# churchill-lab/gbrs

Measured on AMD Instinct MI355X. Metric: EM iterations/s (EMASE Model 4, 40M reads x 8 haplotypes x 120k isoforms per GPU), higher is better.
Workload: dtype f64

## Files before the change

### gbrs_amd/_lib.py

```python
from __future__ import annotations

import ctypes as C
import os

_HERE = os.path.dirname(os.path.abspath(__file__))
LIB_PATH = os.environ.get("GBRS_TUNING_LIB") or os.path.join(_HERE, "libgbrs_hip.so")

EXPORTS = [
    "gbrs_last_error", "gbrs_abi_version", "gbrs_device_count", "gbrs_warm_up",
    "gbrs_em_create", "gbrs_em_create_device", "gbrs_em_create_masked", "gbrs_em_create_masked_device", "gbrs_em_set_initial_values", "gbrs_em_prepare", "gbrs_em_step", "gbrs_em_run",
    "gbrs_em_set_groups", "gbrs_em_step_model", "gbrs_em_posterior",
    "gbrs_em_resample", "gbrs_em_weights", "gbrs_em_resample_info",
    "gbrs_em_bootstrap_begin", "gbrs_em_bootstrap_add", "gbrs_em_bootstrap_get",
    "gbrs_em_get", "gbrs_em_set_theta", "gbrs_em_group_sums", "gbrs_em_estep_partial",
    "gbrs_em_finish_step", "gbrs_em_prepare_partial", "gbrs_em_finish_prepare", "gbrs_em_stream",
    "gbrs_em_set_stream",
    "gbrs_em_sync", "gbrs_em_pair_begin", "gbrs_em_pair_check", "gbrs_em_pair_status", "gbrs_em_info", "gbrs_em_fold_counts", "gbrs_em_tile_cut", "gbrs_em_gather_mstep", "gbrs_em_tile_shapes",
    "gbrs_alignment_counts",
    "gbrs_counts_create", "gbrs_counts_get", "gbrs_counts_destroy", "gbrs_em_destroy",
    "gbrs_shard_plan", "gbrs_shard_index", "gbrs_shard_gather",
    "gbrs_hmm_create", "gbrs_hmm_set_expression", "gbrs_hmm_set_eprob", "gbrs_hmm_run",
    "gbrs_hmm_get", "gbrs_hmm_info", "gbrs_hmm_destroy",
    "gbrs_grid_knots", "gbrs_hmm_set_grid", "gbrs_hmm_grid", "gbrs_hmm_grid_info", "gbrs_hmm_sample_paths", "gbrs_hmm_sample_info",
    "gbrs_hmm_diagnostics", "gbrs_hmm_pair_posterior", "gbrs_hmm_diagnostics_info",
    "gbrs_hmm_set_panel", "gbrs_hmm_match", "gbrs_hmm_match_info",
    "gbrs_hmm_set_snps", "gbrs_hmm_impute", "gbrs_hmm_impute_info", "gbrs_hmm_impute_times",
    "gbrs_hmm_loglik", "gbrs_hmm_loglik_tables", "gbrs_hmm_loglik_info", "gbrs_interpolate", "gbrs_genoprob_dosage",
    "gbrs_ri_transition_tables", "gbrs_alignment_spec",
    "gbrs_scan_create", "gbrs_scan_destroy", "gbrs_scan_append", "gbrs_scan_append_hmm", "gbrs_scan_prepare", "gbrs_scan_run",
    "gbrs_scan_info", "gbrs_scan_permute", "gbrs_scan_perm_info",
    "gbrs_scan_set_snps", "gbrs_scan_snp_dosage", "gbrs_scan_snps", "gbrs_scan_snp_info",
    "gbrs_scan_mediate", "gbrs_scan_mediate_info",
    "gbrs_scan_effects", "gbrs_scan_effects_info", "gbrs_scan_run_support",
    "gbrs_compress_create", "gbrs_compress_get", "gbrs_compress_destroy",
    "gbrs_bam_open", "gbrs_bam_references", "gbrs_bam_set_reference_map", "gbrs_bam_convert", "gbrs_bam_get",
    "gbrs_bam_scan_records", "gbrs_bam_destroy",
    "gbrs_ecset_create", "gbrs_ecset_add_bam", "gbrs_ecset_add_bam_pair", "gbrs_ecset_sizes", "gbrs_ecset_get", "gbrs_ecset_destroy",
    "gbrs_matops_create", "gbrs_matops_intersect", "gbrs_matops_append_rows", "gbrs_matops_keep_unique_rows",
    "gbrs_matops_mask_columns", "gbrs_matops_sizes", "gbrs_matops_get", "gbrs_matops_destroy",
    "gbrs_matops_shared_counts", "gbrs_matops_shared_counts_get", "gbrs_matops_shared_counts_info",
# ... 134 lines not shown
        "gbrs_em_resample": [vp, u64, u32],
        "gbrs_em_weights": [vp, vp],
        "gbrs_em_resample_info": [vp, C.POINTER(u64), C.POINTER(u64), C.POINTER(u32)],
        "gbrs_em_bootstrap_begin": [vp, i64, vp, vp],
        "gbrs_em_bootstrap_add": [vp, vp, vp, vp, vp],
        "gbrs_em_bootstrap_get": [vp, i32, C.POINTER(u32), vp, vp, vp, vp, vp, vp, vp, vp],
        "gbrs_em_get": [vp, vp, vp],
        "gbrs_em_set_theta": [vp, vp],
        "gbrs_em_group_sums": [vp, i64, vp, vp, i32, vp],
        "gbrs_em_estep_partial": [vp, pp, C.POINTER(u64)],
        "gbrs_em_finish_step": [vp, C.POINTER(dbl)],
        "gbrs_em_prepare_partial": [vp, pp, C.POINTER(u64)],
        "gbrs_em_finish_prepare": [vp, dbl],
        "gbrs_em_sync": [vp],
        "gbrs_em_pair_begin": [vp, vp, i32],
        "gbrs_em_pair_check": [vp, vp, dbl],
        "gbrs_em_pair_status": [vp, vp, C.POINTER(i32), C.POINTER(i32), vp, i32],
        "gbrs_em_set_stream": [vp, vp],
        "gbrs_em_info": [vp, C.POINTER(EmInfo)],
        "gbrs_em_fold_counts": [vp, C.POINTER(u64), C.POINTER(u64)],
        "gbrs_em_tile_cut": [vp, C.POINTER(u32), C.POINTER(u32)],
        "gbrs_em_gather_mstep": [vp, C.POINTER(u32)],
        "gbrs_em_tile_shapes": [vp, vp, vp, u64],
        "gbrs_alignment_counts": [u64, u32, u32, pp, pp, vp, vp, u32, i32, vp, vp, vp],
        "gbrs_counts_create": [u64, u32, u32, pp, pp, vp, i32, pp],
        "gbrs_counts_get": [vp, vp, u32, vp, vp, vp],
        "gbrs_counts_destroy": [vp],
        "gbrs_em_destroy": [vp],
        "gbrs_shard_plan": [u64, u32, u32, pp, pp, i32, i32, vp],
        "gbrs_shard_index": [u64, u32, u32, pp, pp, u64, u64, i32, pp, vp],
        "gbrs_shard_gather": [u64, u32, u32, pp, pp, u64, u64, u32, pp, i32, vp, pp, pp, C.POINTER(u64)],
        "gbrs_hmm_create": [i32, i32, vp, vp, pp, i32, pp],
        "gbrs_hmm_set_expression": [vp, i32, pp, pp, pp, dbl, dbl],
        "gbrs_hmm_set_eprob": [vp, i32, pp],
        "gbrs_hmm_run": [vp],
        "gbrs_hmm_get": [vp, i32, i32, vp, vp, vp, vp, vp, vp, vp, vp],
        "gbrs_hmm_info": [vp, C.POINTER(HmmInfo)],
        "gbrs_hmm_destroy": [vp],
        "gbrs_grid_knots": [i32, vp, i32, vp, vp, vp],
        "gbrs_hmm_set_grid": [vp, vp, pp, vp, pp],
        "gbrs_hmm_grid": [vp, i32, vp, vp],
        "gbrs_hmm_grid_info": [vp, C.POINTER(i64), C.POINTER(dbl)],
        "gbrs_hmm_set_panel": [vp, i32, pp],
        "gbrs_hmm_match": [vp, i32, vp, vp],
        "gbrs_hmm_match_info": [vp, C.POINTER(i32), vp, C.POINTER(dbl), C.POINTER(u64)],
        "gbrs_hmm_set_snps": [vp, vp, pp, vp, pp, pp],
# ... 49 lines not shown
        "gbrs_matops_sizes": [vp, C.POINTER(u64), vp, C.POINTER(u32)],
        "gbrs_matops_get": [vp, pp, pp],
        "gbrs_matops_destroy": [vp],
        "gbrs_matops_shared_counts": [vp, vp, u32, C.POINTER(u64)],
        "gbrs_matops_shared_counts_get": [vp, vp, vp, vp],
        "gbrs_matops_shared_counts_info": [vp, C.POINTER(u64), C.POINTER(u64), C.POINTER(u64), C.POINTER(u32),
                                           C.POINTER(u64), C.POINTER(u64), C.POINTER(dbl)],
        "gbrs_tensor_create": [u64, u32, u32, pp, pp, pp, vp, i32, pp],
        "gbrs_tensor_set_groups": [vp, i64, vp, vp],
        "gbrs_tensor_reset": [vp],
        "gbrs_tensor_multiply": [vp, i32, vp, u64],
        "gbrs_tensor_multiply_tensor": [vp, vp],
        "gbrs_tensor_normalize": [vp, i32],
        "gbrs_tensor_sum_reads": [vp, vp],
        "gbrs_tensor_sum_loci": [vp, vp],
        "gbrs_tensor_copy": [vp, pp],
        "gbrs_tensor_values": [vp, u32, vp, vp, u64],
        "gbrs_tensor_set_values": [vp, u32, vp, u64],
        "gbrs_tensor_nnz": [vp, vp],
        "gbrs_tensor_destroy": [vp],
    }
    sigs.update(_host_signatures())
    for name, args in sigs.items():
        if name in ("gbrs_em_fold_counts", "gbrs_em_tile_cut", "gbrs_em_gather_mstep", "gbrs_em_tile_shapes") and os.environ.get("GBRS_TUNING_LIB") and not hasattr(lib, name):
            continue
        fn = getattr(lib, name)
        fn.restype = i32
        fn.argtypes = args
    lib.gbrs_em_stream.restype = vp
    lib.gbrs_em_stream.argtypes = [vp]
    if lib.gbrs_abi_version() != 5:
        raise ImportError("libgbrs_hip.so ABI version mismatch")
    _lib = lib
    return lib


def _host_signatures():
    vp, i32, u32, u64, i64, dbl = C.c_void_p, C.c_int, C.c_uint32, C.c_uint64, C.c_int64, C.c_double
    return {
        "gbrs_format_double": [dbl, C.c_char_p],
        "gbrs_decode_chunks": [C.c_char_p, i64, vp, vp, vp, vp, u64, u32, u64, i32, i32, vp, i32],
        "gbrs_inflate_backend": [],
        "gbrs_zip_directory": [vp, u64, u64, vp, vp, vp, vp, vp, vp, u64, C.POINTER(u64), C.POINTER(u64)],
        "gbrs_npz_stack": [vp, u64, i64, vp, vp, vp, vp, vp, vp, u64, u64, vp, vp, i32],
        "gbrs_zip_read_members": [vp, u64, i64, vp, vp, vp, vp, vp, vp, i32],
        "gbrs_parse_number_table": [C.c_char_p, i64, i64, i32, vp],
        "gbrs_parse_length_table": [C.c_char_p, i64, C.c_char_p, vp, i64, C.c_char_p, vp, i32, dbl, vp],
# ... 52 lines not shown
```

### gbrs_amd/csrc/em.hip

```cpp
#include "common.h"
#include "em_layout.h"
#include "em_step.h"

#include <algorithm>
#include <chrono>
#include <cmath>
#include <cstdlib>

namespace gbrs {


struct EmScalars {
    double s_prev, s_new;
    double err_sum;
    double pc_before, pc_after;
    int stop;
    int iters_done;
    int float_error;
    int ticket;
};

constexpr int RED_BLOCKS = 256;
constexpr int RED_THREADS = 256;

// ... 1915 lines not shown
    *tile_words = em->layout == 1 ? em->tl.cut_tile_words : 0;
    return GBRS_OK;
}

int gbrs_em_gather_mstep(gbrs_em_t *em, uint32_t *taken) {
    if (!em || !taken) return fail(GBRS_ERR_INVALID, "NULL argument");
    *taken = em_gather_route(em) ? 1u : 0u;
    return GBRS_OK;
}

int gbrs_em_tile_shapes(gbrs_em_t *em, uint32_t *n_batches, uint32_t *dict_entries, uint64_t n) {
    if (!em || !n_batches || !dict_entries) return fail(GBRS_ERR_INVALID, "NULL argument");
    if (em->layout != 1 || n != em->tl.n_tiles) return fail(GBRS_ERR_INVALID, "n is not the handle's number of tiles");
    (void)hipSetDevice(em->device);
    std::vector<TileHdr> hdr(n);
    if (n) GBRS_HIP_CHECK(hipMemcpy(hdr.data(), em->tl.tiles.p, n * sizeof(TileHdr), hipMemcpyDeviceToHost));
    for (uint64_t t = 0; t < n; ++t) {
        n_batches[t] = hdr[t].n_batches;
        dict_entries[t] = hdr[t].dict_count();
    }
    return GBRS_OK;
}

int gbrs_counts_create(uint64_t R, uint32_t L, uint32_t H, const uint32_t *const *indptr,
                       const uint32_t *const *indices, const double *count, int device, gbrs_counts_t **out) {
    if (!out) return fail(GBRS_ERR_INVALID, "out is NULL");
    *out = nullptr;
    if (H < 1 || H > 32 || L < 1 || R < 1 || R > 0xFFFFFFFFull || !indptr || !indices)
        return fail(GBRS_ERR_INVALID, "The shape must be a tuple of three positive integers (H <= 32, R < 2^32).");
    GBRS_TRY(select_device(device));
    gbrs_counts *c = new gbrs_counts();
    struct Guard { gbrs_counts *p; ~Guard() { if (p) gbrs_counts_destroy(p); } } guard{c};
    c->device = device;
    c->R = R; c->L = L; c->H = H;
    GBRS_HIP_CHECK(hipStreamCreateWithFlags(&c->s, hipStreamDefault));
    GBRS_TRY(upload_csc(R, L, H, indptr, indices, false, c->ent_row, c->col_ptr, c->n));
    if (count) {
        GBRS_TRY(c->d_count.alloc(R));
        GBRS_HIP_CHECK(hipMemcpy(c->d_count.p, count, R * sizeof(double), hipMemcpyHostToDevice));
    }
    GBRS_HIP_CHECK(hipDeviceSynchronize());
    GBRS_TRY(check_row_ids(c->n, c->ent_row.p, R, c->s));
    c->work = counts_work_new();
    guard.p = nullptr;
    *out = c;
    return GBRS_OK;
// ... 226 lines not shown
```

### gbrs_amd/csrc/em_layout.h

```cpp
#pragma once
#include "common.h"
#include "em_plan.h"

#include <vector>

namespace gbrs {

#ifndef GBRS_TILE_THREADS
#define GBRS_TILE_THREADS 512
#endif
constexpr int TILE_THREADS = GBRS_TILE_THREADS;
constexpr int TILE_WAVES = TILE_THREADS / 64;
#ifndef GBRS_TILE_CAP
#define GBRS_TILE_CAP 32768
#endif
#ifndef GBRS_TILE_WORDS
#define GBRS_TILE_WORDS 2048
#endif
constexpr int TILE_WORDS = GBRS_TILE_WORDS, TILE_WORDS_MAX = GBRS_TILE_CAP - 64, TILE_ROUNDS_MIN = 1;
static_assert(TILE_WORDS <= TILE_WORDS_MAX, "a tile's padded words must fit the dictionary sort");
__host__ __device__ constexpr int pos_bits(int H) { return H <= 8 ? 5 : 3; }
__host__ __device__ constexpr int max_row_words(int H) { return 1 << pos_bits(H); }
#ifndef GBRS_LDS_DOUBLES
#define GBRS_LDS_DOUBLES 3072
// ... 45 lines not shown
    double *theta_new;
    double *tot_prev, *tot_new;
    double *msums;
    uint32_t cap;
    double *acc_cur, *acc_next;
    const uint32_t *gdest, *gdest_b, *gdest_list;
    uint32_t pending;
};

struct TileLayout {
    uint64_t n_pairs = 0;
    uint64_t n_rows_in = 0;
    uint64_t n_rows = 0;
    uint64_t n_folded = 0;
    uint64_t n_folded_two = 0;
    uint64_t n_long = 0;
    uint64_t n_tiles = 0, n_batches = 0, n_slots = 0, n_heavy = 0, n_light = 0;
    uint32_t d_max = 0;
    uint32_t cut_passes = 0;
    uint32_t cut_tile_words = 0;
    bool weighted = false;
    bool deterministic = false;
    bool all_one_word = false;

    DevBuf<uint32_t> words;
    DevBuf<TileHdr> tiles;
    DevBuf<uint32_t> dict;
    DevBuf<double> word_weight;
    DevBuf<double> row_weight;
    DevBuf<uint32_t> slot_ptr;
    DevBuf<uint32_t> slot_list;
    DevBuf<uint32_t> heavy_loci;
    DevBuf<uint32_t> light_loci;
    DevBuf<uint32_t> heavy_range, light_range;
    DevBuf<uint32_t> slot_dest;
    DevBuf<uint8_t> locus_class;
    DevBuf<double> partials;
    DevBuf<uint64_t> long_ptr;
    DevBuf<uint32_t> long_loc, long_mask;
    DevBuf<double> long_weight;
    DevBuf<double> acc_extra;
    bool keep_row_ids = false;
    DevBuf<uint32_t> word_row;
    DevBuf<uint32_t> long_row;
    uint32_t n_sets = 0;
    uint64_t n_dest_rows = 0;
// ... 87 lines not shown
```

### gbrs_amd/csrc/em_layout.hip

```cpp
#include "em_layout.h"
#include "prim.h"

#include <algorithm>

namespace gbrs {
namespace {



struct BuildFlags {
    unsigned int duplicate;
    unsigned int dict_overflow;
    unsigned int bad_row;
    unsigned int n_long;
    unsigned int long_pairs;
};

constexpr int KEY_ITERS = 32, KEY_SPAN = 64 * KEY_ITERS;
__global__ void __launch_bounds__(256)
make_keys_kernel(uint64_t n, uint32_t ncols, uint32_t L, uint64_t R, unsigned row_shift,
                 const uint64_t *__restrict__ col_ptr, const uint32_t *__restrict__ ent_row,
                 uint64_t *__restrict__ keys, BuildFlags *flags, uint32_t view_h = 0) {
    const int lane = threadIdx.x & 63;
    const uint64_t base = ((uint64_t)blockIdx.x * 4 + (threadIdx.x >> 6)) * KEY_SPAN;
// ... 513 lines not shown

__global__ void permute_rows_kernel(uint64_t m_rows, const uint32_t *__restrict__ perm, const uint32_t *__restrict__ hrow,
                                    const uint32_t *__restrict__ npm, const double *__restrict__ weight,
                                    const uint32_t *__restrict__ repeat, uint32_t *__restrict__ hrow2,
                                    uint32_t *__restrict__ npm2, double *__restrict__ weight2,
                                    uint32_t *__restrict__ repeat2) {
    const uint64_t i = (uint64_t)blockIdx.x * blockDim.x + threadIdx.x;
    if (i >= m_rows) return;
    const uint32_t m = perm[i];
    hrow2[i] = hrow[m];
    npm2[i] = npm[m];
    if (weight) weight2[i] = weight[m];
    if (repeat) repeat2[i] = repeat[m];
}

__global__ void tile_start_kernel(uint64_t m_rows, uint64_t n_tiles, const uint32_t *__restrict__ tflag,
                                  const uint32_t *__restrict__ tincl, uint32_t *__restrict__ tile_row) {
    const uint64_t m = (uint64_t)blockIdx.x * blockDim.x + threadIdx.x;
    if (m == 0) tile_row[n_tiles] = (uint32_t)m_rows;
    if (m >= m_rows || !tflag[m]) return;
    tile_row[tincl[m] - 1] = (uint32_t)m;
}

__global__ void tile_pad_kernel(uint64_t n_tiles, int streams, const uint32_t *__restrict__ tile_row,
                                const uint32_t *__restrict__ npm, uint32_t *__restrict__ rowpad,
                                uint32_t *__restrict__ nbatch, uint32_t *__restrict__ n_one, uint32_t *__restrict__ n_two) {
    const uint64_t t = (uint64_t)blockIdx.x * blockDim.x + threadIdx.x;
    if (t >= n_tiles) return;
    uint32_t off = 0, one = 0, two = 0;
    const uint32_t end = tile_row[t + 1];
    uint32_t m = tile_row[t];
    while (m < end) {
        const uint32_t cnt = npm[m];
        if (streams && cnt <= 32u && (64u % cnt) == 0u) {
            uint32_t e = m + 1;
            while (e < end && npm[e] == cnt) ++e;
            const uint32_t n = e - m, G = 64u / cnt, B = (n + G - 1) / G;
            off = (off + 63u) & ~63u;
            if (cnt == 1u && off == 0u) one = B;
            if (cnt == 2u && off == one * 64u) two = B;
            for (uint32_t k = 0; k < n; ++k) rowpad[m + k] = off + (k % B) * 64u + (k / B) * cnt;
            off += B * 64u;
            m = e;
        } else {
            if ((off & 63u) + cnt > 64u) off = (off + 63u) & ~63u;
            rowpad[m] = off;
            off += cnt;
            ++m;
        }
    }
    nbatch[t] = (off + 63u) >> 6;
    n_one[t] = one;
    n_two[t] = two;
}

__global__ void tile_pair_keys_kernel(uint64_t m_rows, const uint32_t *__restrict__ tincl, const uint32_t *__restrict__ hrow,
                                      const uint32_t *__restrict__ rowstart, const uint32_t *__restrict__ ploc,
                                      const uint32_t *__restrict__ wordoff, uint64_t *__restrict__ keys) {
    const uint64_t m = (uint64_t)blockIdx.x * blockDim.x + threadIdx.x;
    if (m >= m_rows) return;
    const uint64_t t = tincl[m] - 1;
    const uint32_t r = hrow[m], p0 = rowstart[r], cnt = rowstart[r + 1] - p0, o = wordoff[m];
    for (uint32_t j = 0; j < cnt; ++j) keys[o + j] = (t << 32) | ploc[p0 + j];
}
// ... 43 lines not shown
        uint32_t lo = 0, hi = th.dict_count();
        while (lo < hi) {
            const uint32_t mid = (lo + hi) >> 1;
            if (d[mid] < l) lo = mid + 1; else hi = mid;
        }
        uint32_t w = pmask[p0 + j] | (j << H) | ((cnt - 1 - j) << (H + PB)) | (lo << (H + 2 * PB));
        if (cnt == 2u && th.n_two() != 0u) w = pmask[p0 + j] | (lo << (H + 2 * PB));
        if (repeat && (cnt == 1u || (cnt == 2u && th.n_two() != 0u))) w |= (repeat[m] - 1u) << H;
        words[base + j] = w;
        if (word_weight) word_weight[base + j] = row_weight[m];
        if (word_row) word_row[base + j] = row_orig[r];
    }
}

__global__ void fill_one_word_cells_kernel(uint64_t n_tiles, uint32_t H, const TileHdr *__restrict__ hdr,
                                           uint32_t *__restrict__ words) {
    const uint64_t i = (uint64_t)blockIdx.x * blockDim.x + threadIdx.x;
    if (i >= n_tiles * 64) return;
    const TileHdr th = hdr[i >> 6];
    for (int run = 0; run < 2; ++run) {
        const uint32_t B = run == 0 ? th.n_one : th.n_two();
        if (B < 2) continue;
        uint32_t *w = words + ((uint64_t)th.batch_base + (run == 0 ? 0u : th.n_one)) * 64 + (i & 63u);
        if (w[0] == 0u || w[(uint64_t)(B - 1) * 64] != 0u) continue;
        uint32_t b = B - 1;
        while (w[(uint64_t)(b - 1) * 64] == 0u) --b;
        const uint32_t fill = w[(uint64_t)(b - 1) * 64] & ~((1u << (H + 2 * pos_bits(H))) - 1u);
        for (; b < B; ++b) w[(uint64_t)b * 64] = fill;
    }
}

__global__ void iota_kernel(uint64_t n, uint32_t *__restrict__ v) {
    const uint64_t i = (uint64_t)blockIdx.x * blockDim.x + threadIdx.x;
    if (i < n) v[i] = (uint32_t)i;
}

__global__ void dest_count_kernel(uint64_t ns, uint32_t L, const uint32_t *__restrict__ dict, const uint32_t *__restrict__ set_ptr,
                                  uint32_t *__restrict__ cnt) {
    const uint64_t i = (uint64_t)blockIdx.x * blockDim.x + threadIdx.x;
    if (i >= ns) return;
    const uint32_t id = dict[i];
    cnt[i] = id < L ? 1u : 1u + (set_ptr[id - L + 1] - set_ptr[id - L]);
}

__global__ void dest_emit_kernel(uint64_t ns, uint32_t L, const uint32_t *__restrict__ dict, const uint32_t *__restrict__ set_ptr,
                                 const uint32_t *__restrict__ members, const uint32_t *__restrict__ eoff,
                                 uint32_t *__restrict__ eloc, uint32_t *__restrict__ eidx, uint32_t *__restrict__ slot_dest,
                                 uint32_t *__restrict__ dest_list) {
    const uint64_t i = (uint64_t)blockIdx.x * blockDim.x + threadIdx.x;
    if (i >= ns) return;
    const uint32_t id = dict[i], o = eoff[i];
// ... 881 lines not shown
    b.mark("7b-d release");
    GBRS_TRY(hrow2.alloc(M)); GBRS_TRY(npm2.alloc(M));
    if (out.weighted) GBRS_TRY(weight2.alloc(M));
    if (fold) GBRS_TRY(repeat2.alloc(M));
    hipLaunchKernelGGL(permute_rows_kernel, dim3(grid_for(M)), dim3(256), 0, s, M, perm.p, lr.hrow.p, t.npm.p,
                       out.weighted ? out.row_weight.p : (const double *)nullptr, fold ? lr.repeat.p : (const uint32_t *)nullptr,
                       hrow2.p, npm2.p, out.weighted ? weight2.p : (double *)nullptr, fold ? repeat2.p : (uint32_t *)nullptr);
    if (fold) GBRS_HIP_CHECK(hipMemcpyAsync(lr.repeat.p, repeat2.p, M * 4, hipMemcpyDeviceToDevice, s));
    GBRS_HIP_CHECK(hipMemcpyAsync(lr.hrow.p, hrow2.p, M * 4, hipMemcpyDeviceToDevice, s));
    GBRS_HIP_CHECK(hipMemcpyAsync(t.npm.p, npm2.p, M * 4, hipMemcpyDeviceToDevice, s));
    if (out.weighted)
        GBRS_HIP_CHECK(hipMemcpyAsync(out.row_weight.p, weight2.p, M * 8, hipMemcpyDeviceToDevice, s));
    GBRS_TRY(exclusive_scan(sc, t.npm.p, t.wordoff.p, M, s));
    GBRS_HIP_CHECK(hipStreamSynchronize(s));
    return GBRS_OK;
}

struct TileParts {
    DevBuf<uint32_t> rowpad, nbatch, n_one, n_two, batch_base, dict_base;
    uint32_t NB = 0, NS = 0;
    void release() { dict_base.release(); batch_base.release(); nbatch.release(); n_one.release(); n_two.release(); rowpad.release(); }
};

int pad_rows(Build &b, TileLayout &out, const Tiles &t, TileParts &tp, uint64_t M, const EmPlan &plan) {
    hipStream_t s = b.s;
    const uint64_t T = t.T;
    GBRS_TRY(tp.rowpad.alloc(M)); GBRS_TRY(tp.nbatch.alloc(T)); GBRS_TRY(tp.n_one.alloc(T)); GBRS_TRY(tp.n_two.alloc(T));
    GBRS_TRY(tp.batch_base.alloc(T));
    hipLaunchKernelGGL(tile_pad_kernel, dim3(grid_for(T, 64)), dim3(64), 0, s, T, plan.row_order == 2 ? 1 : 0, t.tile_row.p, t.npm.p,
                       tp.rowpad.p, tp.nbatch.p, tp.n_one.p, tp.n_two.p);
    if (out.weighted) GBRS_HIP_CHECK(hipMemsetAsync(tp.n_one.p, 0, T * 4, s));
    if (!plan.counted_pairs) GBRS_HIP_CHECK(hipMemsetAsync(tp.n_two.p, 0, T * 4, s));
    GBRS_TRY(scan_total(b.sc, tp.nbatch.p, tp.batch_base.p, T, tp.NB, s));
    out.n_batches = tp.NB;
    return GBRS_OK;
}

int tile_dictionaries(Build &b, TileLayout &out, const RowPairs &rp, const LayoutRows &lr, const Tiles &t, TileParts &tp) {
    hipStream_t s = b.s;
    const uint64_t M = lr.M, T = t.T;
    GBRS_TRY(tp.dict_base.alloc(T));
    uint32_t W = 0;
    GBRS_TRY(fetch_last_plus(t.wordoff.p, t.npm.p, M, W, s));
    DevBuf<uint64_t> dkey, dkey2;
    DevBuf<uint32_t> dflag, dpos;
    GBRS_TRY(dkey.alloc(W)); GBRS_TRY(dkey2.alloc(W)); GBRS_TRY(dflag.alloc(W)); GBRS_TRY(dpos.alloc(W));
    hipLaunchKernelGGL(tile_pair_keys_kernel, dim3(grid_for(M)), dim3(256), 0, s, M, t.tincl.p, lr.hrow.p, rp.rowstart.p, rp.ploc.p,
                       t.wordoff.p, dkey.p);
    GBRS_TRY(sort_keys64(b.sc, dkey.p, dkey2.p, W, 32 + bits_for(T), s));
    hipLaunchKernelGGL(dict_flag_kernel, dim3(grid_for(W)), dim3(256), 0, s, (uint64_t)W, dkey2.p, dflag.p);
    GBRS_TRY(scan_total(b.sc, dflag.p, dpos.p, W, tp.NS, s));
    out.n_slots = tp.NS;
    GBRS_TRY(out.tiles.alloc(T));
// ... 214 lines not shown
        if (plan.group_sets) GBRS_TRY(mask_group_sets(b, out, rp, plan));
        stg.mark("3c mask-group sets");
    }
    SortedRows rows;
    LayoutRows lr;
    GBRS_TRY(order_rows(b, out, rp, rows, L_in + out.n_sets, H));
    stg.mark("4 order rows");
    GBRS_TRY(merge_rows(b, out, rp, rows, lr, count, plan));
    out.all_one_word = false;
    stg.mark("5 merge");
    if (rows.n_long) GBRS_TRY(long_rows(b, out, rp, rows, count, keep_row_ids, plan));
    rows.srow.release();
    if (!keep_row_ids) rp.row_orig.release();
    if (lr.M == 0) { GBRS_HIP_CHECK(hipStreamSynchronize(s)); return GBRS_OK; }
    stg.mark("6 long rows");
    Tiles tiles;
    TileParts parts;
    GBRS_TRY(cut_tiles(b, out, rp, lr, tiles, plan));
    stg.mark("7 tiles");
    if (plan.row_order != 0) GBRS_TRY(order_rows_in_tiles(b, out, lr, tiles, plan.row_order == 1));
    tiles.dnew.release();
    tiles.tflag.release();
    stg.mark("7b row order");
    GBRS_TRY(pad_rows(b, out, tiles, parts, lr.M, plan));
    stg.mark("8 padding");
    GBRS_TRY(tile_dictionaries(b, out, rp, lr, tiles, parts));
    stg.mark("9 dictionaries");
    GBRS_TRY(emit_words(b, out, rp, lr, tiles, parts, keep_row_ids, plan));
    parts.release(); tiles.release(); lr.release(); rp.release();
    out.row_weight.release();
    if (plan.reorder_tiles && tiles.T > 1) GBRS_TRY(reorder_tiles(out, tiles.T));
    stg.mark("10 words");
    GBRS_TRY(inverted_index(b, out, parts.NS, L_in, H));
    stg.mark("11 inverted index");
    GBRS_TRY(heavy_light_lists(out, L_in, s));
    stg.mark("12 heavy / light lists");
    GBRS_HIP_CHECK(hipGetLastError());
    return GBRS_OK;
}

}

namespace gbrs {
namespace {

__global__ void __launch_bounds__(256)
row_hist_kernel(uint64_t n, const uint32_t *__restrict__ ent_row, uint32_t *__restrict__ cnt) {
// ... 78 lines not shown
```

### gbrs_amd/csrc/em_plan.h

```cpp
#pragma once

#include <algorithm>
#include <cstdint>
#include <cstdlib>

#include "../../include/gbrs_hip.h"

namespace gbrs {


struct EmTuning {
    struct Int {
        bool set = false;
        int v = 0;
        bool is(int x) const { return set && v == x; }
        bool nonzero() const { return set && v != 0; }
    };
    int dict_cap = 0;
    Int locus_sets;
    Int group_sets;
    uint32_t set_min_rows = 192;
    Int run_words;
    int tile_words = 0;
    bool tile_cut = true;
    int tile_target = 0;
    bool tile_order = true;
    bool half_loci = false;
    bool persistent = false;
    unsigned persistent_groups = 0;
    bool no_phase_split = false;
    uint32_t resample_cut = 256;
    bool no_fused_mstep = false;
    bool no_float_check = false;
    bool no_gather_mstep = false;
};

namespace em_env {
inline EmTuning::Int integer(const char *name) {
    EmTuning::Int i;
    if (const char *e = std::getenv(name); e) { i.set = true; i.v = std::atoi(e); }
    return i;
}
template <typename T>
inline void at_least(const char *name, int lo, T &v) {
    if (const char *e = std::getenv(name); e && std::atoi(e) >= lo) v = (T)std::atoi(e);
}
}

inline EmTuning em_tuning_from_env() {
    using namespace em_env;
    EmTuning t;
    at_least("GBRS_TUNING_DICT_CAP", 1, t.dict_cap);
    t.locus_sets = integer("GBRS_TUNING_LOCUS_SETS");
    t.group_sets = integer("GBRS_TUNING_GROUP_SETS");
    at_least("GBRS_TUNING_SET_MIN_ROWS", 1, t.set_min_rows);
    t.run_words = integer("GBRS_TUNING_RUN_WORDS");
    at_least("GBRS_TUNING_TILE_WORDS", 64, t.tile_words);
    t.tile_cut = !integer("GBRS_TUNING_TILE_CUT").is(0);
    at_least("GBRS_TUNING_TILE_TARGET", 1, t.tile_target);
    t.tile_order = !integer("GBRS_TUNING_TILE_ORDER").is(0);
    t.half_loci = integer("GBRS_TUNING_HALF_LOCI").nonzero();
    t.persistent = integer("GBRS_TUNING_PERSISTENT").nonzero();
    at_least("GBRS_TUNING_PERSISTENT_GROUPS", 1, t.persistent_groups);
    t.no_phase_split = integer("GBRS_TUNING_NO_PHASE_SPLIT").nonzero();
    at_least("GBRS_TUNING_RESAMPLE_CUT", 1, t.resample_cut);
    t.no_fused_mstep = integer("GBRS_TUNING_NO_FUSED_MSTEP").nonzero();
    t.no_float_check = integer("GBRS_TUNING_NO_FLOAT_CHECK").set;
    t.no_gather_mstep = integer("GBRS_TUNING_NO_GATHER_MSTEP").nonzero();
    return t;
}


struct EmDictLimits {
    uint32_t max_row_words = 0;
    uint32_t index_limit = 0;
    uint32_t lds_doubles = 0;
    uint32_t det_cap = 0;
};

struct EmShape {
    uint32_t H = 0, L = 0;
    uint64_t R = 0, N = 0;
    uint32_t flags = 0;
    bool counts_given = false;
    int n_cu = 0;
    uint32_t tile_words = 0, tile_words_max = 0, tile_rounds_min = 1;
    uint32_t err_blocks = 0;
    EmDictLimits dict;
    EmDictLimits dict_half;
};

// ... 14 lines not shown
    bool group_sets = false;
    bool group_sets_forced = false;
    int sets_forced = -1;
    uint32_t set_min_rows = 192;
    bool counted_pairs = false;
    bool fold = false;
    int fold_mode = 3;
    bool fold_forced = false;
    unsigned per_cu = 3;
    uint64_t places = 0;
    uint32_t tile_words = 0, tile_words_cap = 0;
    uint32_t tile_words_forced = 0;
    bool exact_cut = false;
    uint64_t tile_target = 0;
    bool tile_target_forced = false;
    bool reorder_tiles = true;
    uint32_t d_max = 0, dseg = 0;
    bool dict_room = false;
    uint32_t persist_groups = 0;
    uint32_t lead_mask = ~0u;
    uint32_t resample_cut = 256;
    bool no_fused_mstep = false, no_float_check = false;
    bool no_gather_mstep = false;
};

inline uint64_t em_tile_target(uint64_t places, unsigned side_by_side, uint32_t err_blocks, int forced) {
    if (forced > 0) return (uint64_t)forced;
    const uint64_t n = std::max<uint64_t>(places / std::max(side_by_side, 1u), 1);
    return n > err_blocks ? n - err_blocks : n;
}

inline EmPlan em_plan(const EmShape &s, const EmTuning &t) {
    EmPlan p;
    const uint32_t f = s.flags;
    p.merge = (f & GBRS_EM_MERGE_IDENTICAL_ROWS) != 0;
    p.deterministic = (f & GBRS_EM_DETERMINISTIC) != 0;
    p.weighted = em_weighted(f, s.counts_given);
    p.side_by_side = (f & GBRS_EM_SIDE_BY_SIDE) ? 2u : 1u;
    p.no_fused_mstep = t.no_fused_mstep;
    p.no_float_check = t.no_float_check;
    p.no_gather_mstep = t.no_gather_mstep;
    if ((f & GBRS_EM_RESAMPLE) && s.counts_given) p.resample_cut = t.resample_cut;
    p.tiled = !(f & GBRS_EM_LAYOUT_CSC) && s.H <= 16 && s.N < 0xFFFFFFFFull;
    p.tH = s.H;
    p.tL = s.L;
    if (!p.tiled) return p;

    if (f & GBRS_EM_FORCE_INTERLEAVE) p.row_order = 1;
    else if (f & GBRS_EM_NO_STREAMS) p.row_order = (p.weighted && !(f & GBRS_EM_NO_INTERLEAVE)) ? 1 : 0;
    if (s.H == 16 && t.half_loci && !p.weighted && !p.deterministic && (uint64_t)s.L * 2 < (1u << 27)) p.view = 2;
    p.tH = s.H / p.view;
    p.tL = s.L * p.view;
    const EmDictLimits &d = p.view == 2 ? s.dict_half : s.dict;

    p.locus_sets = !(f & GBRS_EM_NO_LOCUS_SETS) && !p.weighted;
    p.whole_row_sets = p.locus_sets && t.locus_sets.is(1);
    if (t.locus_sets.set) p.sets_forced = t.locus_sets.v != 0;
    p.group_sets = p.locus_sets && !t.group_sets.is(0);
    p.group_sets_forced = t.group_sets.is(1);
    p.set_min_rows = t.set_min_rows;

    p.counted_pairs = p.row_order == 2 && !p.weighted && !p.deterministic && p.view == 1 &&
                      (p.tH == 1 || p.tH == 2 || p.tH == 4 || p.tH == 8);
    p.fold = !(f & GBRS_EM_NO_RUN_WORDS) && p.counted_pairs && !t.run_words.is(0);
    p.fold_mode = t.run_words.is(1) ? 2 : 3;
    p.fold_forced = t.run_words.set;

    p.per_cu = (p.weighted || p.tH > 8) ? 2u : 3u;
    const unsigned n_cu = (unsigned)std::max(s.n_cu, 1);
    p.places = (uint64_t)s.tile_rounds_min * p.per_cu * n_cu;
    p.tile_words = s.tile_words;
    p.tile_words_cap = p.weighted ? std::min<uint32_t>(s.tile_words_max, 16320) : s.tile_words_max;
    if (t.tile_words) p.tile_words_forced = std::min<uint32_t>((uint32_t)t.tile_words, s.tile_words_max);
    p.exact_cut = t.tile_cut && !p.tile_words_forced;
    p.tile_target = em_tile_target(p.places, p.side_by_side, s.err_blocks, t.tile_target);
    p.tile_target_forced = t.tile_target > 0;
    p.reorder_tiles = t.tile_order;

    p.d_max = std::min<uint32_t>(1024, d.lds_doubles / p.tH);
    p.d_max = std::min(p.d_max, d.index_limit);
    if (p.deterministic) p.d_max = std::min(p.d_max, d.det_cap);
    if (t.dict_cap > (int)d.max_row_words) p.d_max = std::min(p.d_max, (uint32_t)t.dict_cap);
    p.dict_room = p.d_max > d.max_row_words;
    p.dseg = p.dict_room ? p.d_max - d.max_row_words : 0;

    unsigned groups = p.per_cu * n_cu / p.side_by_side;
    if (t.persistent_groups) groups = t.persistent_groups;
    p.persist_groups = t.persistent ? std::max(groups, 1u) : 0u;
    p.lead_mask = t.no_phase_split ? 0u : ~0u;
// ... 8 lines not shown
}

constexpr int TILE_CUT_PASSES = 3;
inline bool em_take_exact_cut(const EmPlan &p, uint64_t total_words) {
    if (!p.exact_cut) return false;
    return p.tile_target_forced || (total_words + p.tile_target - 1) / p.tile_target <= p.tile_words_cap;
}
inline uint32_t em_cut_clamp(const EmPlan &p, uint64_t words) {
    return (uint32_t)std::min<uint64_t>(std::max<uint64_t>((words + 63) & ~63ull, p.tile_words), p.tile_words_cap);
}
inline uint32_t em_cut_tile_words(const EmPlan &p, uint64_t total_words) {
    return em_cut_clamp(p, (total_words + p.tile_target - 1) / p.tile_target);
}
inline uint32_t em_cut_rescale(const EmPlan &p, uint32_t tile_words, uint64_t tiles) {
    if (tiles <= p.tile_target) return tile_words;
    return std::max(tile_words, em_cut_clamp(p, ((uint64_t)tile_words * tiles + p.tile_target - 1) / p.tile_target));
}

inline bool em_take_fold(const EmPlan &p, uint64_t words_in, uint64_t folded) {
    if (p.fold_forced) return true;
    return folded * 100 >= words_in * 15 && (words_in - folded) * p.side_by_side / p.places >= (uint64_t)p.tile_words;
}

inline bool em_use_whole_row_sets(const EmPlan &p, uint64_t P, uint64_t P2, uint64_t L, uint64_t V) {
    if (p.sets_forced >= 0) return p.sets_forced != 0;
    return P2 * 100 <= P * 85 && P2 >= 100 * (L + V) && V <= 2 * L;
}

inline bool em_group_sets_fit(const EmPlan &p, uint64_t V, uint64_t L) { return V * 2 <= L || p.group_sets_forced; }
inline bool em_use_group_sets(const EmPlan &p, uint64_t P, uint64_t P2) { return p.group_sets_forced || P2 * 100 <= P * 95; }

}
```

### gbrs_amd/engine.py

```python
from __future__ import annotations

import ctypes as C

import numpy as np

from . import _lib


def _allowed_array(allowed, L):
    al = np.ascontiguousarray(allowed, dtype=np.uint32)
    if al.shape != (L,):
        raise RuntimeError('allowed must hold one haplotype bit mask per locus')
    return al


class EmEngine:
    def __init__(self, handle, shape, keepalive=None):
        self._h = handle
        self.shape = shape
        self._keep = keepalive

    @classmethod
    def from_host(cls, R, L, H, indptr, indices, count=None, eff_len=None, device=0, flags=0, allowed=None):
        lib = _lib.load()
# ... 97 lines not shown
        return inf

    def fold_counts(self):
        one, two = C.c_uint64(0), C.c_uint64(0)
        _lib.check(_lib.load().gbrs_em_fold_counts(self._h, C.byref(one), C.byref(two)))
        return int(one.value), int(two.value)

    def tile_cut(self):
        passes, words = C.c_uint32(0), C.c_uint32(0)
        _lib.check(_lib.load().gbrs_em_tile_cut(self._h, C.byref(passes), C.byref(words)))
        return int(passes.value), int(words.value)

    def gather_mstep(self):
        taken = C.c_uint32(0)
        _lib.check(_lib.load().gbrs_em_gather_mstep(self._h, C.byref(taken)))
        return bool(taken.value)

    def tile_shapes(self):
        n = int(self.info().num_tiles)
        batches, entries = np.zeros(n, np.uint32), np.zeros(n, np.uint32)
        _lib.check(_lib.load().gbrs_em_tile_shapes(self._h, batches.ctypes.data, entries.ctypes.data, n))
        return batches, entries

    def _partial(self, fn):
        p = C.c_void_p()
        n = C.c_uint64(0)
        _lib.check(fn(self._h, C.byref(p), C.byref(n)))
        return p.value, int(n.value)

    def estep_partial(self):
        return self._partial(_lib.load().gbrs_em_estep_partial)

    def prepare_partial(self):
        return self._partial(_lib.load().gbrs_em_prepare_partial)

    def finish_step(self, want_err=True):
        err = C.c_double(0.0)
        _lib.check(_lib.load().gbrs_em_finish_step(self._h, C.byref(err) if want_err else None))
        return err.value

    def finish_prepare(self, pseudocount=0.0):
        _lib.check(_lib.load().gbrs_em_finish_prepare(self._h, float(pseudocount)))

    def sync(self):
        _lib.check(_lib.load().gbrs_em_sync(self._h))

# ... 18 lines not shown
```

### include/gbrs_hip.h

```cpp
#ifndef GBRS_HIP_H
#define GBRS_HIP_H

#include <stdint.h>

#ifdef __cplusplus
extern "C" {
#endif

#define GBRS_ABI_VERSION 5

enum gbrs_status {
    GBRS_OK = 0,
    GBRS_ERR_INVALID = -1,
    GBRS_ERR_HIP = -2,
    GBRS_ERR_NO_DEVICE = -3,
    GBRS_ERR_FLOAT = -4,
    GBRS_ERR_UNSUPPORTED = -5,
    GBRS_ERR_STATE = -6
};

const char *gbrs_last_error(void);
int gbrs_abi_version(void);
int gbrs_device_count(void);
int gbrs_warm_up(int device);
// ... 87 lines not shown
    uint64_t num_device_rows;
    uint64_t num_device_words;
    uint64_t bytes_per_iter;
    uint64_t algorithmic_bytes;
    double   last_estep_ms;
    double   last_step_ms;
    uint32_t num_loci, num_haps;
    uint32_t layout;
    uint32_t num_folded_rows;
    uint64_t num_tiles;
    uint64_t num_slots;
    uint64_t num_long_rows;
    uint64_t num_heavy_loci;
    uint64_t num_light_loci;
    uint64_t estep_bytes;
    uint64_t retained_build_bytes;
    uint64_t num_locus_sets;
} gbrs_em_info_t;
int gbrs_em_info(gbrs_em_t *em, gbrs_em_info_t *info);
int gbrs_em_fold_counts(gbrs_em_t *em, uint64_t *one_word_reads, uint64_t *two_word_reads);
int gbrs_em_tile_cut(gbrs_em_t *em, uint32_t *passes, uint32_t *tile_words);
int gbrs_em_gather_mstep(gbrs_em_t *em, uint32_t *taken);
int gbrs_em_tile_shapes(gbrs_em_t *em, uint32_t *n_batches, uint32_t *dict_entries, uint64_t n);

int gbrs_alignment_counts(uint64_t num_rows, uint32_t num_loci, uint32_t num_haps,
                          const uint32_t *const *indptr, const uint32_t *const *indices,
                          const double *count, const int32_t *locus_group, uint32_t num_out_loci,
                          int device, double *aln_counts, double *allele_unique, double *locus_unique);

typedef struct gbrs_counts gbrs_counts_t;
int gbrs_counts_create(uint64_t num_rows, uint32_t num_loci, uint32_t num_haps,
                       const uint32_t *const *indptr, const uint32_t *const *indices,
                       const double *count, int device, gbrs_counts_t **out);
int gbrs_counts_get(gbrs_counts_t *c, const int32_t *locus_group, uint32_t num_out_loci,
                    double *aln_counts, double *allele_unique, double *locus_unique);
int gbrs_counts_destroy(gbrs_counts_t *c);

int gbrs_shard_plan(uint64_t num_rows, uint32_t num_loci, uint32_t num_haps,
                    const uint32_t *const *indptr, const uint32_t *const *indices,
                    int world, int device, uint64_t *bounds);
int gbrs_shard_index(uint64_t num_rows, uint32_t num_loci, uint32_t num_haps,
                     const uint32_t *const *indptr, const uint32_t *const *indices,
                     uint64_t r0, uint64_t r1, int device,
                     uint32_t *const *indptr_out, uint64_t *nnz_out);
int gbrs_shard_gather(uint64_t num_rows, uint32_t num_loci, uint32_t num_haps,
                      const uint32_t *const *indptr, const uint32_t *const *indices,
// ... 282 lines not shown
```

Measured before the change: 26750.

## Align same-locus row runs into stripes in the tiled E-step layout

Adds a stripe layout for the leading one-word and two-word row streams of each tile. A head flag marks rows whose locus differs from the previous row, and runs are padded to 2-, 4- or 8-batch boundaries so each lane sees fewer locus changes between consecutive batches. Stripe width is picked automatically when the padding overhead stays under a cap, or forced through an environment variable. The padding fill now also rewrites interior empty slots. A census API is added to count locus transitions. In exchange it adds padded cells and build-time work.

```diff
diff --git a/gbrs_amd/_lib.py b/gbrs_amd/_lib.py
--- a/gbrs_amd/_lib.py
+++ b/gbrs_amd/_lib.py
@@ -15,7 +15,7 @@
     "gbrs_em_get", "gbrs_em_set_theta", "gbrs_em_group_sums", "gbrs_em_estep_partial",
     "gbrs_em_finish_step", "gbrs_em_prepare_partial", "gbrs_em_finish_prepare", "gbrs_em_stream",
     "gbrs_em_set_stream",
-    "gbrs_em_sync", "gbrs_em_pair_begin", "gbrs_em_pair_check", "gbrs_em_pair_status", "gbrs_em_info", "gbrs_em_fold_counts", "gbrs_em_tile_cut", "gbrs_em_gather_mstep", "gbrs_em_tile_shapes",
+    "gbrs_em_sync", "gbrs_em_pair_begin", "gbrs_em_pair_check", "gbrs_em_pair_status", "gbrs_em_info", "gbrs_em_fold_counts", "gbrs_em_tile_cut", "gbrs_em_gather_mstep", "gbrs_em_tile_shapes", "gbrs_em_stripe_census",
     "gbrs_alignment_counts",
     "gbrs_counts_create", "gbrs_counts_get", "gbrs_counts_destroy", "gbrs_em_destroy",
     "gbrs_shard_plan", "gbrs_shard_index", "gbrs_shard_gather",
@@ -196,6 +196,7 @@
         "gbrs_em_tile_cut": [vp, C.POINTER(u32), C.POINTER(u32)],
         "gbrs_em_gather_mstep": [vp, C.POINTER(u32)],
         "gbrs_em_tile_shapes": [vp, vp, vp, u64],
+        "gbrs_em_stripe_census": [vp, u32, vp],
         "gbrs_alignment_counts": [u64, u32, u32, pp, pp, vp, vp, u32, i32, vp, vp, vp],
         "gbrs_counts_create": [u64, u32, u32, pp, pp, vp, i32, pp],
         "gbrs_counts_get": [vp, vp, u32, vp, vp, vp],
@@ -291,7 +292,7 @@
     }
     sigs.update(_host_signatures())
     for name, args in sigs.items():
-        if name in ("gbrs_em_fold_counts", "gbrs_em_tile_cut", "gbrs_em_gather_mstep", "gbrs_em_tile_shapes") and os.environ.get("GBRS_TUNING_LIB") and not hasattr(lib, name):
+        if name in ("gbrs_em_fold_counts", "gbrs_em_tile_cut", "gbrs_em_gather_mstep", "gbrs_em_tile_shapes", "gbrs_em_stripe_census") and os.environ.get("GBRS_TUNING_LIB") and not hasattr(lib, name):
             continue
         fn = getattr(lib, name)
         fn.restype = i32
diff --git a/gbrs_amd/csrc/em.hip b/gbrs_amd/csrc/em.hip
--- a/gbrs_amd/csrc/em.hip
+++ b/gbrs_amd/csrc/em.hip
@@ -1961,6 +1961,41 @@
     return GBRS_OK;
 }
 
+int gbrs_em_stripe_census(gbrs_em_t *em, uint32_t S, uint64_t *out) {
+    if (!em || !out) return fail(GBRS_ERR_INVALID, "NULL argument");
+    for (int k = 0; k < 6; ++k) out[k] = 0;
+    if (em->layout != 1 || em->tl.n_tiles == 0) return GBRS_OK;
+    (void)hipSetDevice(em->device);
+    const TileLayout &tl = em->tl;
+    std::vector<TileHdr> hdr(tl.n_tiles);
+    std::vector<uint32_t> words((size_t)tl.n_batches * 64);
+    GBRS_HIP_CHECK(hipMemcpy(hdr.data(), tl.tiles.p, hdr.size() * sizeof(TileHdr), hipMemcpyDeviceToHost));
+    if (!words.empty()) GBRS_HIP_CHECK(hipMemcpy(words.data(), tl.words.p, words.size() * 4, hipMemcpyDeviceToHost));
+    const uint32_t H = em->plan.tH, shift = H + 2 * pos_bits((int)H), hmask = (1u << H) - 1u;
+    for (const TileHdr &th : hdr) {
+        const uint32_t nb = th.n_batches, lead = std::min<uint32_t>(th.n_one + th.n_two(), nb);
+        if ((uint64_t)th.batch_base + nb > tl.n_batches) return fail(GBRS_ERR_STATE, "a tile header is out of range");
+        const uint32_t *w = words.data() + (size_t)th.batch_base * 64;
+        for (uint32_t b = 0; b < lead; ++b)
+            for (int l = 0; l < 64; ++l) out[4] += (w[(size_t)b * 64 + l] & hmask) == 0u;
+        out[0] += lead;
+        for (int wave = 0; wave < TILE_WAVES; ++wave) {
+            const uint32_t b0 = (uint32_t)(((uint64_t)nb * wave) / TILE_WAVES), b1 = (uint32_t)(((uint64_t)nb * (wave + 1)) / TILE_WAVES);
+            if (b0 < b1 && b0 < lead) ++out[1];
+            for (uint32_t b = b0 + 1; b < std::min(b1, lead); ++b) {
+                uint32_t lanes = 0;
+                for (int l = 0; l < 64; ++l) lanes += (w[(size_t)b * 64 + l] >> shift) != (w[(size_t)(b - 1) * 64 + l] >> shift);
+                if (!lanes) continue;
+                ++out[2];
+                out[3] += lanes;
+                const uint32_t first = b < th.n_one ? 0u : th.n_one;
+                if (S != 0 && (b - first) % S != 0) ++out[5];
+            }
+        }
+    }
+    return GBRS_OK;
+}
+
 int gbrs_counts_create(uint64_t R, uint32_t L, uint32_t H, const uint32_t *const *indptr,
                        const uint32_t *const *indices, const double *count, int device, gbrs_counts_t **out) {
     if (!out) return fail(GBRS_ERR_INVALID, "out is NULL");
diff --git a/gbrs_amd/csrc/em_layout.h b/gbrs_amd/csrc/em_layout.h
--- a/gbrs_amd/csrc/em_layout.h
+++ b/gbrs_amd/csrc/em_layout.h
@@ -91,6 +91,7 @@
     bool weighted = false;
     bool deterministic = false;
     bool all_one_word = false;
+    bool stripes = false;
 
     DevBuf<uint32_t> words;
     DevBuf<TileHdr> tiles;
diff --git a/gbrs_amd/csrc/em_layout.hip b/gbrs_amd/csrc/em_layout.hip
--- a/gbrs_amd/csrc/em_layout.hip
+++ b/gbrs_amd/csrc/em_layout.hip
@@ -559,9 +559,33 @@
     tile_row[tincl[m] - 1] = (uint32_t)m;
 }
 
+__global__ void stripe_head_kernel(uint64_t m_rows, const uint32_t *__restrict__ npm, const uint32_t *__restrict__ hrow,
+                                   const uint32_t *__restrict__ rowstart, const uint32_t *__restrict__ ploc,
+                                   uint8_t *__restrict__ head) {
+    const uint64_t m = (uint64_t)blockIdx.x * blockDim.x + threadIdx.x;
+    if (m >= m_rows) return;
+    const uint32_t cnt = npm[m];
+    uint8_t h = 1;
+    if (m > 0 && cnt <= 2u && npm[m - 1] == cnt) {
+        const uint32_t a = rowstart[hrow[m - 1]], b = rowstart[hrow[m]];
+        h = (ploc[a] != ploc[b] || (cnt == 2u && ploc[a + 1] != ploc[b + 1])) ? 1 : 0;
+    }
+    head[m] = h;
+}
+
+__device__ __forceinline__ uint32_t stripe_cells(const uint8_t *__restrict__ head, uint32_t n, uint32_t S) {
+    uint32_t c = 0;
+    for (uint32_t k = 0; k < n; ++k) {
+        if (head[k]) c = (c + S - 1u) & ~(S - 1u);
+        ++c;
+    }
+    return (c + S - 1u) & ~(S - 1u);
+}
+
 __global__ void tile_pad_kernel(uint64_t n_tiles, int streams, const uint32_t *__restrict__ tile_row,
                                 const uint32_t *__restrict__ npm, uint32_t *__restrict__ rowpad,
-                                uint32_t *__restrict__ nbatch, uint32_t *__restrict__ n_one, uint32_t *__restrict__ n_two) {
+                                uint32_t *__restrict__ nbatch, uint32_t *__restrict__ n_one, uint32_t *__restrict__ n_two,
+                                const uint8_t *__restrict__ head, int stripes_one, int stripes_two) {
     const uint64_t t = (uint64_t)blockIdx.x * blockDim.x + threadIdx.x;
     if (t >= n_tiles) return;
     uint32_t off = 0, one = 0, two = 0;
@@ -572,11 +596,29 @@
         if (streams && cnt <= 32u && (64u % cnt) == 0u) {
             uint32_t e = m + 1;
             while (e < end && npm[e] == cnt) ++e;
-            const uint32_t n = e - m, G = 64u / cnt, B = (n + G - 1) / G;
+            const uint32_t n = e - m, G = 64u / cnt;
+            uint32_t B = (n + G - 1) / G;
             off = (off + 63u) & ~63u;
-            if (cnt == 1u && off == 0u) one = B;
-            if (cnt == 2u && off == one * 64u) two = B;
-            for (uint32_t k = 0; k < n; ++k) rowpad[m + k] = off + (k % B) * 64u + (k / B) * cnt;
+            const bool lead_one = cnt == 1u && off == 0u, lead_two = cnt == 2u && off == one * 64u;
+            uint32_t S = 0;
+            if (head && (lead_one || lead_two)) {
+                const int forced = lead_one ? stripes_one : stripes_two;
+                S = forced >= 0 ? (uint32_t)forced : em_stripe_pick(forced, n, stripe_cells(head + m, n, 4u), stripe_cells(head + m, n, 2u));
+            }
+            if (S != 0u) {
+                B = (stripe_cells(head + m, n, S) + G - 1) / G;
+                B = (B + S - 1u) & ~(S - 1u);
+                uint32_t c = 0;
+                for (uint32_t k = 0; k < n; ++k) {
+                    if (head[m + k]) c = (c + S - 1u) & ~(S - 1u);
+                    rowpad[m + k] = off + (c % B) * 64u + (c / B) * cnt;
+                    ++c;
+                }
+            } else {
+                for (uint32_t k = 0; k < n; ++k) rowpad[m + k] = off + (k % B) * 64u + (k / B) * cnt;
+            }
+            if (lead_one) one = B;
+            if (lead_two) two = B;
             off += B * 64u;
             m = e;
         } else {
@@ -666,11 +708,12 @@
         const uint32_t B = run == 0 ? th.n_one : th.n_two();
         if (B < 2) continue;
         uint32_t *w = words + ((uint64_t)th.batch_base + (run == 0 ? 0u : th.n_one)) * 64 + (i & 63u);
-        if (w[0] == 0u || w[(uint64_t)(B - 1) * 64] != 0u) continue;
-        uint32_t b = B - 1;
-        while (w[(uint64_t)(b - 1) * 64] == 0u) --b;
-        const uint32_t fill = w[(uint64_t)(b - 1) * 64] & ~((1u << (H + 2 * pos_bits(H))) - 1u);
-        for (; b < B; ++b) w[(uint64_t)b * 64] = fill;
+        uint32_t fill = 0;
+        for (uint32_t b = 0; b < B; ++b) {
+            const uint32_t x = w[(uint64_t)b * 64];
+            if (x & ((1u << H) - 1u)) fill = x & ~((1u << (H + 2 * pos_bits(H))) - 1u);
+            else if (x != fill) w[(uint64_t)b * 64] = fill;
+        }
     }
 }
 
@@ -1598,13 +1641,23 @@
     void release() { dict_base.release(); batch_base.release(); nbatch.release(); n_one.release(); n_two.release(); rowpad.release(); }
 };
 
-int pad_rows(Build &b, TileLayout &out, const Tiles &t, TileParts &tp, uint64_t M, const EmPlan &plan) {
+int pad_rows(Build &b, TileLayout &out, const RowPairs &rp, const LayoutRows &lr, const Tiles &t, TileParts &tp,
+             const EmPlan &plan) {
     hipStream_t s = b.s;
-    const uint64_t T = t.T;
+    const uint64_t T = t.T, M = lr.M;
     GBRS_TRY(tp.rowpad.alloc(M)); GBRS_TRY(tp.nbatch.alloc(T)); GBRS_TRY(tp.n_one.alloc(T)); GBRS_TRY(tp.n_two.alloc(T));
     GBRS_TRY(tp.batch_base.alloc(T));
+    DevBuf<uint8_t> head;
+    uint32_t W = 0;
+    if (plan.counted_pairs && (plan.stripes_one != 0 || plan.stripes_two != 0)) GBRS_TRY(fetch_last_plus(t.wordoff.p, t.npm.p, M, W, s));
+    out.stripes = em_take_stripes(plan, W);
+    if (out.stripes) {
+        GBRS_TRY(head.alloc(M));
+        hipLaunchKernelGGL(stripe_head_kernel, dim3(grid_for(M)), dim3(256), 0, s, M, t.npm.p, lr.hrow.p, rp.rowstart.p, rp.ploc.p, head.p);
+    }
     hipLaunchKernelGGL(tile_pad_kernel, dim3(grid_for(T, 64)), dim3(64), 0, s, T, plan.row_order == 2 ? 1 : 0, t.tile_row.p, t.npm.p,
-                       tp.rowpad.p, tp.nbatch.p, tp.n_one.p, tp.n_two.p);
+                       tp.rowpad.p, tp.nbatch.p, tp.n_one.p, tp.n_two.p, out.stripes ? head.p : (const uint8_t *)nullptr,
+                       plan.stripes_one, plan.stripes_two);
     if (out.weighted) GBRS_HIP_CHECK(hipMemsetAsync(tp.n_one.p, 0, T * 4, s));
     if (!plan.counted_pairs) GBRS_HIP_CHECK(hipMemsetAsync(tp.n_two.p, 0, T * 4, s));
     GBRS_TRY(scan_total(b.sc, tp.nbatch.p, tp.batch_base.p, T, tp.NB, s));
@@ -1865,7 +1918,7 @@
     tiles.dnew.release();
     tiles.tflag.release();
     stg.mark("7b row order");
-    GBRS_TRY(pad_rows(b, out, tiles, parts, lr.M, plan));
+    GBRS_TRY(pad_rows(b, out, rp, lr, tiles, parts, plan));
     stg.mark("8 padding");
     GBRS_TRY(tile_dictionaries(b, out, rp, lr, tiles, parts));
     stg.mark("9 dictionaries");
diff --git a/gbrs_amd/csrc/em_plan.h b/gbrs_amd/csrc/em_plan.h
--- a/gbrs_amd/csrc/em_plan.h
+++ b/gbrs_amd/csrc/em_plan.h
@@ -33,6 +33,7 @@
     bool no_fused_mstep = false;
     bool no_float_check = false;
     bool no_gather_mstep = false;
+    int stripes_one = -1, stripes_two = -1;
 };
 
 namespace em_env {
@@ -44,6 +45,10 @@
 template <typename T>
 inline void at_least(const char *name, int lo, T &v) {
     if (const char *e = std::getenv(name); e && std::atoi(e) >= lo) v = (T)std::atoi(e);
+}
+inline int stripe_value(const char *e) {
+    const int v = std::atoi(e);
+    return (v == 0 && *e == '0') || v == 2 || v == 4 || v == 8 ? v : -1;
 }
 }
 
@@ -67,6 +72,11 @@
     t.no_fused_mstep = integer("GBRS_TUNING_NO_FUSED_MSTEP").nonzero();
     t.no_float_check = integer("GBRS_TUNING_NO_FLOAT_CHECK").set;
     t.no_gather_mstep = integer("GBRS_TUNING_NO_GATHER_MSTEP").nonzero();
+    if (const char *e = std::getenv("GBRS_TUNING_STRIPES"); e) {
+        t.stripes_one = t.stripes_two = stripe_value(e);
+        for (const char *c = e; *c; ++c)
+            if (*c == ',') { t.stripes_two = stripe_value(c + 1); break; }
+    }
     return t;
 }
 
@@ -127,6 +137,8 @@
     uint32_t resample_cut = 256;
     bool no_fused_mstep = false, no_float_check = false;
     bool no_gather_mstep = false;
+    int stripes_one = 0, stripes_two = 0;
+    bool stripes_forced = false;
 };
 
 inline uint64_t em_tile_target(uint64_t places, unsigned side_by_side, uint32_t err_blocks, int forced) {
@@ -170,6 +182,11 @@
     p.fold = !(f & GBRS_EM_NO_RUN_WORDS) && p.counted_pairs && !t.run_words.is(0);
     p.fold_mode = t.run_words.is(1) ? 2 : 3;
     p.fold_forced = t.run_words.set;
+    if (p.counted_pairs) {
+        p.stripes_one = t.stripes_one;
+        p.stripes_two = t.stripes_two;
+        p.stripes_forced = t.stripes_one > 0 || t.stripes_two > 0;
+    }
 
     p.per_cu = (p.weighted || p.tH > 8) ? 2u : 3u;
     const unsigned n_cu = (unsigned)std::max(s.n_cu, 1);
@@ -224,6 +241,20 @@
     return folded * 100 >= words_in * 15 && (words_in - folded) * p.side_by_side / p.places >= (uint64_t)p.tile_words;
 }
 
+inline bool em_take_stripes(const EmPlan &p, uint64_t words) {
+    if (!p.counted_pairs || (p.stripes_one == 0 && p.stripes_two == 0)) return false;
+    if (p.stripes_forced) return true;
+    return words * p.side_by_side / p.places >= (uint64_t)p.tile_words;
+}
+constexpr uint32_t STRIPE_CAP_NUM = 1, STRIPE_CAP_DEN = 4;
+constexpr bool em_stripe_fits(uint64_t cells, uint64_t words) {
+    return cells * STRIPE_CAP_DEN <= words * (STRIPE_CAP_DEN + STRIPE_CAP_NUM);
+}
+constexpr uint32_t em_stripe_pick(int forced, uint64_t words, uint64_t cells4, uint64_t cells2) {
+    if (forced >= 0) return (uint32_t)forced;
+    return em_stripe_fits(cells4, words) ? 4u : em_stripe_fits(cells2, words) ? 2u : 0u;
+}
+
 inline bool em_use_whole_row_sets(const EmPlan &p, uint64_t P, uint64_t P2, uint64_t L, uint64_t V) {
     if (p.sets_forced >= 0) return p.sets_forced != 0;
     return P2 * 100 <= P * 85 && P2 >= 100 * (L + V) && V <= 2 * L;
diff --git a/gbrs_amd/engine.py b/gbrs_amd/engine.py
--- a/gbrs_amd/engine.py
+++ b/gbrs_amd/engine.py
@@ -143,6 +143,11 @@
         _lib.check(_lib.load().gbrs_em_tile_shapes(self._h, batches.ctypes.data, entries.ctypes.data, n))
         return batches, entries
 
+    def stripe_census(self, S=0):
+        out = np.zeros(6, np.uint64)
+        _lib.check(_lib.load().gbrs_em_stripe_census(self._h, int(S), out.ctypes.data))
+        return out
+
     def _partial(self, fn):
         p = C.c_void_p()
         n = C.c_uint64(0)
diff --git a/include/gbrs_hip.h b/include/gbrs_hip.h
--- a/include/gbrs_hip.h
+++ b/include/gbrs_hip.h
@@ -133,6 +133,7 @@
 int gbrs_em_tile_cut(gbrs_em_t *em, uint32_t *passes, uint32_t *tile_words);
 int gbrs_em_gather_mstep(gbrs_em_t *em, uint32_t *taken);
 int gbrs_em_tile_shapes(gbrs_em_t *em, uint32_t *n_batches, uint32_t *dict_entries, uint64_t n);
+int gbrs_em_stripe_census(gbrs_em_t *em, uint32_t S, uint64_t *out);
 
 int gbrs_alignment_counts(uint64_t num_rows, uint32_t num_loci, uint32_t num_haps,
                           const uint32_t *const *indptr, const uint32_t *const *indices,
```

Result: faster. 29890, median of 6 (+11.7%).
